# SouthPoleTelescope/CosmoMC

Hardware: AMD Instinct MI355X
Metric: fast-param likelihood evals/sec/node (plik_lite_TTTEEE ℓmax=2508); R-1 vs wall-clock (higher is better)
Workload: dtype f64; 1 GPU; plik_lite_TTTEEE + Planck2018 lensing fast-parameter Metropolis step (BASELINE configs[2] minus lowl): GetProposalFast + native plik_lite (613 bins, l<=2508, full binning + quadratic form) + CMBlikes lensing (9 bins, linear correction) + calPlanck prior + accept; walkers_per_gpu=1024, stream_groups=1, global_walkers=1024, nbins=613, lmax=2508, parallelism=walkers sharded over 1 rank(s), no per-step collective

## Files before the change

### cosmomc_amd/csrc/common.h

```cpp
#pragma once

#include <hip/hip_runtime.h>
#include <hip/hip_ext.h>

#include <algorithm>
#include <cstdarg>
#include <cstdint>
#include <cstdio>
#include <map>
#include <memory>
#include <mutex>
#include <stdexcept>
#include <string>
#include <vector>

#include "../../include/cosmomc_amd.h"

namespace cmamd {

struct Error : std::runtime_error {
    int code;
    Error(int c, const std::string &m) : std::runtime_error(m), code(c) {}
};

// ... 146 lines not shown
struct QFSource {
    const double *Ct = nullptr;
    int Np = 0, xcd_map = 0;
    const QFItem *items = nullptr;
    int n_items = 0;
    double *partial = nullptr;
    const double *X = nullptr;
    const double *delta = nullptr;
    unsigned int *counters = nullptr;
    int n_counters = 0;
};

struct SmallGaussDev {
    int nE, nX, has_corr, cal_index;
    double log_cal_prior;
    const int *e_to_x;
    const double *e_main_const, *e_corr_const;
    const double *fidcorr, *chat;
    int ntask;
    const int *trow;
    const int *e_main_t, *e_corr_t;
    const int *wcount;
};
struct SmallGaussLaunch {
    SmallGaussDev d;
    const double *partial;
    const double *nuis;
    long long ld_nuis;
    const double *M;
    double *out;
    int W;
    const unsigned char *row_cal;
    int stage_cal;
};

struct WinCol {
    int field, lo, hi;
    const double *w;
    int row;
    int cal;
};
struct WinStage {
    int kind = 0;
    int cal_index = -1;
    std::vector<WinCol> cols;
    const double *X = nullptr;
    int ld = 0;
};

struct Like {
    virtual ~Like() = default;
    std::string name, tag, nuisance_names;
    int n_nuis = 0;
    std::string derived_names;
    int n_derived = 0;
    virtual void derived_batch(int W, const double *nuis, long long ld_nuis, double *out, long long ld_out,
                               hipStream_t stream) {
        (void)nuis, (void)ld_nuis;
        if (W <= 0 || n_derived <= 0) return;
        if (!out || ld_out < n_derived) fail(CMBL_ERR_ARG, "derived output needs %d columns", n_derived);
        HIP_CHECK(hipMemset2DAsync(out, (size_t)ld_out * 8, 0, (size_t)n_derived * 8, W, stream));
    }
    const double *nuisance_rows(const double *nuis, const void *unread) const {
        if (n_nuis > 0 && !nuis) fail(CMBL_ERR_ARG, "%s needs its %d nuisance parameters", name.c_str(), n_nuis);
        return nuis ? nuis : static_cast<const double *>(unread);
    }
// ... 104 lines not shown
```

### cosmomc_amd/csrc/mhbody.h

```cpp
#pragma once

template <bool ACCEPT, bool PROPOSE>
__device__ __forceinline__ void mh_body(const DevCfg &c, int fast_only, double *hist_row, double *hist_terms, int blk0,
                                        double *lds, int bx, const TailWait *tw = nullptr)
{
    if (c.lean.on) {
        mh_lean<ACCEPT, PROPOSE>(c, hist_row, hist_terms, blk0, lds, bx, tw);
        return;
    }
    const Rows &R = c.rows;
    const int lane = threadIdx.x % MB, grp = threadIdx.x / MB;
    const int wl64 = threadIdx.x & 63, wave = threadIdx.x >> 6, nwave = MH_THREADS / 64;
    const int wb = (blk0 + bx) * MB;
    const int w = wb + lane;
    const bool act = w < c.W;
    const size_t W = c.ld;
    const int nlk = (c.n_like + 1) & ~1;
    const int nd_st = c.stage_R ? R.ND : R.ND - R.RR;
    const int ni_st = c.stage_cyc ? R.NI : R.CYC;
    const int ntd = c.stage_cov ? c.tl.n_dbl : c.tl.covinv;
    double *sd = lds;
    double *lk = sd + (size_t)nd_st * MB;
    double *vc = lk + (size_t)nlk * MB;
    double *tq = vc + (size_t)c.max_blk * MB;
    double *dq = tq + (size_t)c.tq_rows * MB;
    double *td = dq + (size_t)c.def_cap * (QF_GROUPS + 1) * MB;
    int *si = reinterpret_cast<int *>(td + ((ntd + 31) & ~31));
    int *it = si + (size_t)ni_st * MB;
    int *ti = it + (size_t)(c.stage_cyc ? c.all_n : 0) * MB;
    int *oobw = ti + ((c.tl.n_int + 63) & ~63);
    double *zz = reinterpret_cast<double *>(oobw + MB);
    int *ndw = reinterpret_cast<int *>(zz + (size_t)c.np * MB);
    int *i0w = ndw + MB;
    if (threadIdx.x < MB) oobw[threadIdx.x] = 0;
    if (PROPOSE && c.rot_defer && bx == 0 && threadIdx.x == 0)
        c.rot_cnt[2 * (blk0 * MB / 64) + (c.rot_par ^ 1)] = 0;
    const bool skipR = !c.stage_R;
#define SROW(r) ((skipR && (r) >= R.R) ? (r) - R.RR : (r))

    STAMP(0);
// ... 288 lines not shown
    }
    if (PROPOSE && c.pub_on && threadIdx.x < MB && act)
        for (int k = 0; k < 2; k++) {
            const int pc = c.pub_pcal[k];
            const bool rp = si[(size_t)R.PROT * MB + lane] != 0;
            const double v = rp ? __longlong_as_double((long long)TP_PIPE_ROT)
                                : pc >= 0 ? sd[(size_t)(SROW(R.T) + pc) * MB + lane] : 1.0;
            __hip_atomic_store(c.calbuf + (size_t)k * W + w, v, __ATOMIC_RELAXED, __HIP_MEMORY_SCOPE_AGENT);
            __hip_atomic_store(c.calbuf_next + (size_t)k * W + w, __longlong_as_double((long long)TP_PIPE_UNSET),
                               __ATOMIC_RELAXED, __HIP_MEMORY_SCOPE_AGENT);
        }
    if (act) {
        const int nd = ndw[lane], i0 = i0w[lane];
        for (int t = grp; t < nd; t += NV) {
            int p = i0 - 1 - t;
            if (p < 0) p += 97;
            c.sd[(size_t)(R.U + p) * W + w] = sd[(size_t)(R.U + p) * MB + lane];
        }
    }
    if (skipR) {
        stage_out(c.sd, sd, R.C, R.C, R.R, W, wb);
        stage_out(c.sd, sd, R.R, rEnd, R.ND, W, wb);
    } else {
        stage_out(c.sd, sd, R.C, R.C, R.ND, W, wb);
    }
    stage_out(c.si, si, 0, 0, ni_st, W, wb);
    STAMP(5);
#ifdef CMAMD_STAMPS
    asm volatile("s_waitcnt vmcnt(0)" ::: "memory");
    STAMP(6);
#endif
#undef SROW
}
```

### cosmomc_amd/csrc/mhlean.h

```cpp
#pragma once

template <bool ACCEPT, bool PROPOSE>
__device__ __forceinline__ void mh_lean(const DevCfg &c, double *hist_row, double *hist_terms, int blk0, double *lds,
                                        int bx, const TailWait *tw)
{
    const Rows &R = c.rows;
    const LeanCfg &L = c.lean;
    const int lane = threadIdx.x % MB, grp = threadIdx.x / MB;
    const int wl64 = threadIdx.x & 63, wave = threadIdx.x >> 6, nwave = MH_THREADS / 64;
    const int wb = (blk0 + bx) * MB;
    const int w = wb + lane;
    const bool act = w < c.W;
    const size_t W = c.ld;
    const int np = c.np;
    const int nd_lo = R.R, nd_hi = R.ND - R.P;
    double *sd = lds;
    double *sp = sd + (size_t)nd_lo * MB;
    double *dq = sp + (size_t)nd_hi * MB;
    double *zz = dq + (size_t)MAXDEF * (QF_GROUPS + 1) * MB;
    int *si = reinterpret_cast<int *>(zz + (size_t)np * MB);
    int *oobw = si + 8 * MB;
    int *ndw = oobw + MB;
    int *i0w = ndw + MB;
    if (threadIdx.x < MB) oobw[threadIdx.x] = 0;
    if (PROPOSE && c.rot_defer && bx == 0 && threadIdx.x == 0)
        c.rot_cnt[2 * (blk0 * MB / 64) + (c.rot_par ^ 1)] = 0;

    STAMP(0);
    dma_rows_f64(sd, 0, c.sd, 0, nd_lo, W, wb, wl64, wave, nwave);
    dma_rows_f64(sd, nd_lo, c.sd, R.P, nd_hi, W, wb, wl64, wave, nwave);
    dma_rows_i32(si, c.si, 8, W, wb, wl64, wave, nwave);
    constexpr int PG = MAXP / NV;
    double lo[PG], hi[PG], mu[PG], sg[PG];
    const double *td = c.tab_d;
#pragma unroll
    for (int u = 0; u < PG; u++) {
        const int i = grp + u * NV;
        if (ACCEPT && i < np) {
            lo[u] = td[c.tl.pmin + i];
            hi[u] = td[c.tl.pmax + i];
            mu[u] = td[c.tl.pmean + i];
            sg[u] = td[c.tl.pstd + i];
        }
    }
    int pu[PG];
    if (ACCEPT && hist_row) {
#pragma unroll
        for (int u = 0; u < PG; u++) {
            const int i = grp + u * NV;
            if (i < c.n_used) pu[u] = c.tab_i[c.tl.params_used + i];
        }
    }
    if (tw) tail_wait(*tw, wb / 64);
    if (ACCEPT && c.n_def) {
        const int tile = wb / QF_TILE, col = wb % QF_TILE + lane;
        for (int d = 0; d < MAXDEF; d++) {
            if (d >= c.n_def) break;
            const double *tp = c.def_part[d] + (size_t)tile * c.def_items[d] * QF_TILE;
            double *row = dq + (size_t)d * (QF_GROUPS + 1) * MB;
            if (grp < QF_GROUPS) row[(size_t)grp * MB + lane] = qf_group_sum(tp, c.def_items[d], grp, col);
            if (grp == NV - 1) row[(size_t)QF_GROUPS * MB + lane] = (c.def_add[d] && act) ? c.def_add[d][w] : 0.0;
        }
    }
    double lk[MAXLIKE], ct[MAXLIKE];
    if (ACCEPT && grp == 0 && act) {
#pragma unroll
        for (int l = 0; l < MAXLIKE; l++)
            if (l < c.n_like) {
                lk[l] = c.like_terms[(size_t)l * W + w];
                if (hist_terms) ct[l] = c.cur_terms[(size_t)l * W + w];
            }
    }
    STAMP(1);
    asm volatile("s_waitcnt vmcnt(0)" ::: "memory");
    __syncthreads();
    const double *trial_l = sp + (size_t)np * MB + lane;
    if (ACCEPT && act) {
        int oob = 0;
#pragma unroll
        for (int u = 0; u < PG; u++) {
            const int i = grp + u * NV;
            if (i < np) {
                const double qv = trial_l[(size_t)i * MB];
                if (qv > hi[u] || qv < lo[u]) oob = 1;
                double z2 = 0.0;
// ... 142 lines not shown
        c.si[(size_t)R.J97 * W + w] = r.j97;
        c.si[(size_t)R.ISET * W + w] = r.iset;
        ndw[lane] = r.nd < 97 ? r.nd : 97;
        i0w[lane] = i97_0;
    }
    __syncthreads();
    STAMP(12);
    if (!act) return;
    {
        const int nd = ndw[lane], i0 = i0w[lane];
        for (int t = grp; t < nd; t += NV) {
            int p = i0 - 1 - t;
            if (p < 0) p += 97;
            c.sd[(size_t)(R.U + p) * W + w] = sd[(size_t)(R.U + p) * MB + lane];
        }
    }
    for (int i = grp; i < np; i += NV) {
        if (ACCEPT) c.sd[(size_t)(R.P + i) * W + w] = sp[(size_t)i * MB + lane];
        if (PROPOSE) c.sd[(size_t)(R.T + i) * W + w] = sp[(size_t)(np + i) * MB + lane];
    }
    if (ACCEPT && hist_row) {
#pragma unroll
        for (int u = 0; u < PG; u++) {
            const int i = grp + u * NV;
            if (i < c.n_used) hist_row[(size_t)i * c.W + w] = sp[(size_t)pu[u] * MB + lane];
        }
    }
    STAMP(5);
#ifdef CMAMD_STAMPS
    asm volatile("s_waitcnt vmcnt(0)" ::: "memory");
    STAMP(6);
#endif
}
```

### cosmomc_amd/csrc/mhstep.h

```cpp
#pragma once


static constexpr int UNI_WT = 4;

template <bool ACCEPT, bool PROPOSE>
__device__ __forceinline__ void mh_step_body(DevCfg &c, int fast_only, double *hist_row, double *hist_terms,
                                             StepTail &t, const int2 *__restrict__ rows, TailWait &tw, int nmh)
{
    extern __shared__ __attribute__((aligned(16))) double lds[];
    const int2 rr = rows[blockIdx.x >> 3];
    const int lb = rr.y * 8 + (blockIdx.x & 7);
    if (!ACCEPT && blockIdx.x == 0)
        for (int i = threadIdx.x; i < tw.ntiles; i += MH_THREADS) tw.cnt[i] = 0u;
#ifdef CMAMD_STAMPS
    const bool stamp = ACCEPT && threadIdx.x == 0 && blockIdx.x < 2048;
    const int slot = PROPOSE ? 0 : 1;
    if (stamp) {
        unsigned xcc;
        asm volatile("s_getreg_b32 %0, hwreg(HW_REG_XCC_ID)" : "=s"(xcc));
        g_uni_stamps[slot][blockIdx.x][0] = __builtin_amdgcn_s_memrealtime();
        g_uni_stamps[slot][blockIdx.x][2] = xcc & 15;
        g_uni_stamps[slot][blockIdx.x][4] = 0;
        g_uni_stamps[slot][blockIdx.x][5] = 0;
    }
    struct End {
        bool on;
        int role, slot;
        __device__ ~End() {
            if (on) {
                g_uni_stamps[slot][blockIdx.x][3] = __builtin_amdgcn_s_memrealtime();
                g_uni_stamps[slot][blockIdx.x][4] = role + 1;
            }
        }
    } end_{stamp, rr.x, slot};
#endif
    if (rr.x == TAIL_QF) {
        if (lb >= t.nq) return;
        int item_ix, tile;
        qf_place(lb, t.q.src.n_items, t.q.src.xcd_map, item_ix, tile);
        __builtin_amdgcn_s_setprio(2);
        qfs_body(lds, item_ix, tile, t.q);
        tail_arrive(tw, tile);
    } else if (rr.x == TAIL_GAUSS) {
        const int grows = (t.ng + 7) >> 3, q = (lb & 7) * grows + (lb >> 3);
        if (q >= t.ng) return;
        small_gauss_body<UNI_WT, true, true>(t.g, lds, q);
        tail_arrive(tw, q * UNI_WT / 64);
    } else if (rr.x == TAIL_PASS) {
        if (lb >= t.np) return;
        tp_vec_body<2, true, false>(t.tp, t.dl, t.ld_field, t.ld_walker, t.W, reinterpret_cast<char *>(lds), lb);
    } else if (lb < nmh) {
        __builtin_amdgcn_s_setprio(3);
        if (ACCEPT && t.fold_g) {
            small_gauss_body<MB, true, false>(t.g, lds, lb);
            asm volatile("s_waitcnt vmcnt(0)" ::: "memory");
            __syncthreads();
#ifdef CMAMD_STAMPS
            if (threadIdx.x == 0 && blockIdx.x < 2048)
                g_uni_stamps[PROPOSE ? 0 : 1][blockIdx.x][5] = __builtin_amdgcn_s_memrealtime();
#endif
        }
        mh_body<ACCEPT, PROPOSE>(c, fast_only, hist_row, hist_terms, 0, lds, lb, ACCEPT ? &tw : nullptr);
    }
}
```

### cosmomc_amd/csrc/sampler.h

```cpp
#pragma once

#include "common.h"
#include "steptail.h"
#include "theorypass.h"

namespace cmamd {

static constexpr int MAXLIKE = 8;
static constexpr int MAXGROUPS = 8;
static constexpr int MAXDEF = 2;

struct Rows {
    int U = 0;
    int C = 97;
    int G = 98;
    int R = 100;
    int RR;
    int P, T, L, M;
    int ND;
    int I97 = 0, J97 = 1, ISET = 2, FASTIX = 3, NACC = 4;
    int CYCLP = 5;
    int BLKLP = 8;
    int ACCF;
    int PROT;
// ... 87 lines not shown
};

struct LikeSlot {
    cmbl_t *like;
    std::vector<int> nidx;
    TheoryView th;
};

struct PendingDeferred {
    int n = 0;
    int like[MAXDEF], items[MAXDEF];
    const double *part[MAXDEF], *add[MAXDEF];
};

struct PipeStatus {
    int *host = nullptr;
    int *dev = nullptr;
    hipEvent_t ev = nullptr;
    bool pending = false;
    void init();
    void post(hipStream_t stream);
    void post_nothrow(hipStream_t stream);
    void check(bool wait);
    ~PipeStatus() {
        if (host) (void)hipHostFree(host);
        if (ev) (void)hipEventDestroy(ev);
    }
};

struct UnifiedSteps {
    int ready = 0;
    DevBuf S[2][2];
    DevBuf rowcal;
    int qf = -1, g = -1;
    DevBuf cnt;
    size_t cnt_bytes = 0;
    unsigned epoch = 0;
    unsigned epoch_g = 0;
    StepTailPlan plan[3];
    size_t lds = 0;
    bool binned_cache = false;
    void invalidate() { ready = 0; }
};

struct BinCorun {
    int ready = 0;
    DevBuf cal;
    unsigned epoch = 0;
    DevBuf S;
    size_t lds = 0;
    void invalidate() { ready = 0; }
};

}

struct cmbg;

struct cmbs {
    cmamd::DevCfg dc{};
    int W = 0, np = 0, n_used = 0;
    std::vector<int> params_used;
    std::string last_error;
    cmamd::DevBuf rot;
    std::vector<int> rot_par;
    std::vector<int> rot_lp;
    bool rot_fast_any = false;
// ... 88 lines not shown
```

### cosmomc_amd/csrc/sampler.hip

```cpp
#include <algorithm>
#include <cmath>
#include <cstring>

#include <cstdlib>

#include "plikbin.h"
#include "qfs_body.h"
#include "quadform.h"
#include "sampler.h"
#include "smallgauss.h"
#include "theorycalc.h"
#ifdef CMAMD_STAMPS
namespace cmamd {
__device__ unsigned long long g_uni_stamps[2][2048][6];
}
#endif
#include "theorypass_body.h"

namespace cmamd {

static constexpr double LOGZERO = CMBL_LOGZERO;
static constexpr int MAXP = 64;
static constexpr int MAXBLK = 32;
static constexpr int NB = 64;
// ... 86 lines not shown
            }
            __builtin_amdgcn_s_sleep(24);
        }
        cal_s = cl;
    }
    __syncthreads();
    const double cl = cal_s, c2 = cl * cl;
    const bool rot = (unsigned long long)__double_as_longlong(cl) == TP_PIPE_ROT;
    double *out = (rot ? const_cast<double *>(c.bin_S) : c.bin_delta) + (size_t)w * pb.Np;
#pragma unroll
    for (int f = 0; f < 3; f++)
#pragma unroll
        for (int k = 0; k < 2; k++) {
            const int i = pb.fr.b0[f] + (int)threadIdx.x + k * MH_THREADS;
            if (pb.fr.hi[f] >= pb.fr.lo[f] && i < pb.fr.b1[f]) out[i] = rot ? acc[f][k] : pb.X[i] - acc[f][k] / c2;
        }
}

#include "mhstep.h"

template <bool ACCEPT, bool PROPOSE>
__global__ __launch_bounds__(MH_THREADS, 3) void mh_step_kernel(DevCfg c, int fast_only, double *hist_row,
                                                                double *hist_terms, StepTail t,
                                                                const int2 *__restrict__ rows, TailWait tw, int nmh)
{
    mh_step_body<ACCEPT, PROPOSE>(c, fast_only, hist_row, hist_terms, t, rows, tw, nmh);
}

template <bool ACCEPT, bool PROPOSE>
__global__ __launch_bounds__(MH_THREADS, 3) void mh_tail_kernel(DevCfg c, int fast_only, double *hist_row,
                                                                double *hist_terms, StepTail t,
                                                                const int2 *__restrict__ rows, TailWait tw, int nmh)
{
    mh_step_body<ACCEPT, PROPOSE>(c, fast_only, hist_row, hist_terms, t, rows, tw, nmh);
}

#include "mhrot.h"
#include "mhdrag.h"

__global__ void start_kernel(DevCfg c)
{
    const int w = blockIdx.x * blockDim.x + threadIdx.x;
    if (w >= c.W) return;
    const size_t W = c.ld;
    const Tabs t = make_tabs(c, c.tab_i, c.tab_d);
    Col<double> q{c.sd + (size_t)c.rows.T * W + w, c.ld};
    Col<const double> lk{c.like_terms + w, c.ld};
    c.sd[(size_t)c.rows.L * W + w] = target_like(c, t, q, lk);
    for (int l = 0; l < c.n_like; l++) c.cur_terms[(size_t)l * W + w] = lk[l];
    for (int i = 0; i < c.np; i++) c.sd[(size_t)(c.rows.P + i) * W + w] = q[i];
    c.sd[(size_t)c.rows.M * W + w] = 0.0;
    c.si[(size_t)c.rows.NACC * W + w] = 0;
}

__global__ void gather_nuis(const double *trial, int W, int ld, const int *nidx, int n_nuis, double *out)
{
    const int w = blockIdx.x * blockDim.x + threadIdx.x;
    if (w >= W) return;
    for (int k = 0; k < n_nuis; k++) out[(size_t)w * n_nuis + k] = trial[(size_t)nidx[k] * ld + w];
}

struct SparseSet {
    int like[MAXLIKE], nn[MAXLIKE];
    double *nuisc[MAXLIKE];
    int *map[MAXLIKE];
};

// ... 878 lines not shown
    return 0;
}
extern "C" int cmamd_debug_lean(cmbs *s, int on) {
    if (!s) return CMBL_ERR_ARG;
    s->lean_off = !on;
    return 0;
}
extern "C" int cmamd_debug_corun(cmbs *s, int on) {
    if (!s) return -1;
    s->no_corun = !on;
    return 0;
}
extern "C" int cmamd_debug_tail_nosignal(cmbs *s, int on) {
    if (!s) return -1;
    s->handoff_nosignal = on;
    return 0;
}
extern "C" int cmamd_debug_drag_pair(cmbs *s, int on) {
    if (!s) return -1;
    s->no_drag_pair = on == 0;
    return 0;
}
extern "C" int cmamd_debug_drag_hbm(cmbs *s, int on) {
    if (!s) return -1;
    s->drag_hbm = on != 0;
    return 0;
}
extern "C" int cmamd_debug_pipe_status(cmbs *s) {
    if (!s || !s->pipe_status.host) return -1;
    if (hipDeviceSynchronize() != hipSuccess) return -1;
    return *reinterpret_cast<volatile int *>(s->pipe_status.host);
}
extern "C" int cmamd_debug_tail(const cmbs *s) { return s ? s->unified.ready : 0; }
extern "C" int cmamd_debug_fused(const cmbs *s) { return !s ? 0 : s->tpass ? s->tpass->n_items() : -s->tp_why; }
```

### cosmomc_amd/csrc/schedunified.h

```cpp

using StepKernel = void (*)(DevCfg, int, double *, double *, StepTail, const int2 *, TailWait, int);
static const StepKernel step_kernels[2][3] = {
    {mh_step_kernel<false, true>, mh_step_kernel<true, true>, mh_step_kernel<true, false>},
    {mh_step_kernel<false, true>, mh_tail_kernel<true, true>, mh_tail_kernel<true, false>}};
static const char *const step_names[2][3] = {{"mh_step_first", "mh_step_kernel", "mh_step_last"},
                                             {"mh_step_first", "mh_tail_kernel", "mh_tail_last"}};

static bool unified_setup(cmbs *s, int fast_only) {
    if (s->sched_mode == 0 || !fast_only || !s->tpass || s->n_groups != 1 || s->mask_on ||
        (s->dc.rot_defer && s->rot_fast_any) || s->likes.size() != 2 || !s->dlikes.empty())
        return false;
    const TheoryView &P = s->likes[s->tp_like[0]].th;
    if (!s->tpass->vec_ok(P.dl, P.ld_field, P.ld_walker)) return false;
    UnifiedSteps &u = s->unified;
    if (u.ready == s->W) return true;
    if (u.ready == -s->W) return false;
    u.qf = u.g = -1;
    SmallGaussLaunch g{};
    for (int k = 0; k < 2; k++) {
        const int i = s->tp_like[k];
        const WinStage &st = s->tp_stage[k];
        QFSource src;
        if (st.kind == 1 && is_deferred(s, (size_t)i) && s->likes[i].like->like->qf_source(src, s->W, s->like_ws[i].p)) {
            bool all_cal = st.cal_index >= 0;
            for (const WinCol &c : st.cols) all_cal = all_cal && c.cal;
            if (all_cal && st.ld == src.Np) u.qf = k;
        }
        if (st.kind == 0 && small_gauss_on(s, trial_set(s), i, g)) u.g = k;
    }
    if (u.qf < 0 || u.g < 0 || u.qf == u.g) {
        u.ready = -s->W;
        return false;
    }
    const size_t Wp = (size_t)QuadForm::wpad(s->W);
    int rows = 0;
    for (const WinCol &c : s->tp_stage[u.g].cols) rows = std::max(rows, c.row + 1);
    const size_t bytes[2] = {Wp * (size_t)s->tp_stage[u.qf].ld * 8, (size_t)rows * s->W * 8};
    for (int p = 0; p < 2; p++)
        for (int k = 0; k < 2; k++) u.S[p][k].alloc(bytes[k == u.qf ? 0 : 1]);
    std::vector<unsigned char> rc((size_t)rows + 16, 0);
    for (const WinCol &c : s->tp_stage[u.g].cols) rc[c.row] = c.cal ? 1 : 0;
    u.rowcal.alloc(rc.size());
    u.rowcal.upload(rc.data(), rc.size());
    u.cnt_bytes = (Wp / QF_TILE * TW_PAD * 4 + 15) & ~(size_t)15;
    u.cnt.alloc(u.cnt_bytes);
    s->pipe_status.init();
    u.lds = std::max({s->mh_lds, (size_t)QFS_LDS_DOUBLES * 8, (size_t)tp_vec_lds_bytes<2>(),
                      (size_t)small_gauss_lds_doubles<UNI_WT>(g.d.nX) * 8,
                      (size_t)small_gauss_lds_doubles<MB>(g.d.nX) * 8});
    for (auto &ks : step_kernels)
        for (StepKernel k : ks)
            HIP_CHECK(hipFuncSetAttribute((const void *)k, hipFuncAttributeMaxDynamicSharedMemorySize, (int)u.lds));
    for (auto &pl : u.plan) pl.key[0] = -1;
    u.ready = s->W;
    return true;
}

static bool fold_chi2(bool has_pass, int nX) { return has_pass && nX <= MH_THREADS / MB; }

static StepTail make_tail(cmbs *s, int rd, int wr) {
    const UnifiedSteps &u = s->unified;
    StepTail t;
    const int W = s->W;
    t.W = W;
    if (rd >= 0) {
        const int qi = s->tp_like[u.qf];
        Like &Q = *s->likes[qi].like->like;
        if (!Q.qf_source(t.q.src, W, s->like_ws[qi].p)) fail(CMBL_ERR_ARG, "internal: step tail quadratic form");
        t.q.S = u.S[rd][u.qf].as<double>();
        t.q.nuis = s->dc.like_nuis[qi];
        t.q.ld_nuis = std::max(1, Q.n_nuis);
        t.q.cal_index = s->tp_stage[u.qf].cal_index;
        t.q.W = W;
        t.q.Wp = QuadForm::wpad(W);
        t.nq = t.q.src.n_items * (QuadForm::wpad(W) / QF_TILE);
        if (!small_gauss_on(s, trial_set(s), s->tp_like[u.g], t.g)) fail(CMBL_ERR_ARG, "internal: step tail chi^2");
        t.g.partial = u.S[rd][u.g].as<double>();
        t.g.row_cal = u.rowcal.as<unsigned char>();
        t.g.stage_cal = s->tp_stage[u.g].cal_index;
        t.fold_g = fold_chi2(wr >= 0, t.g.d.nX) ? 1 : 0;
        t.ng = t.fold_g ? 0 : (W + UNI_WT - 1) / UNI_WT;
    }
    if (wr >= 0) {
        TPOut o[2];
        fused_outs(s, trial_set(s), o, u.S[wr]);
        t.tp = s->tpass->dev_args(o, W);
        const TheoryView &P = s->likes[s->tp_like[0]].th;
        t.dl = P.dl;
        t.ld_field = P.ld_field;
        t.ld_walker = P.ld_walker;
        t.np = s->tpass->n_blocks();
    }
    return t;
}

static void launch_unified(cmbs *s, hipStream_t stream, bool propose, int rd, int wr, const HistRow &row,
                           int fast_only) {
    UnifiedSteps &u = s->unified;
    const bool accept = rd >= 0;
    StepTail t = make_tail(s, rd, wr);
    DevCfg dc = launch_cfg(s, fast_only, false);
    dc.n_def = accept ? 1 : 0;
    if (accept) {
        dc.def_like[0] = s->tp_like[u.qf];
        dc.def_items[0] = t.q.src.n_items;
        dc.def_part[0] = t.q.src.partial;
        dc.def_add[0] = nullptr;
    }
    TailWait tw{};
    tw.cnt = u.cnt.as<unsigned int>();
    tw.epoch = u.epoch + (accept ? 1u : 0u);
    tw.epoch_g = u.epoch_g + ((accept && !t.fold_g) ? 1u : 0u);
    tw.nq_items = t.q.src.n_items;
    tw.ng = accept ? (s->W + UNI_WT - 1) / UNI_WT : 0;
    tw.gwt = UNI_WT;
    tw.status = s->pipe_status.dev;
    tw.nosignal = s->handoff_nosignal;
    tw.stamp_slot = propose ? 0 : 1;
    tw.ntiles = (int)(u.cnt_bytes / 4);
    const int nmh = (s->W + MB - 1) / MB;
    const int v = accept ? (propose ? 1 : 2) : 0;
    StepTailPlan &pl = u.plan[v];
    if (pl.key[0] != t.nq || pl.key[1] != t.ng || pl.key[2] != t.np) {
        const std::vector<int2> rows = tail_rows(t.nq, t.ng, t.np, nmh);
        pl.d_rows.alloc(rows.size() * sizeof(int2));
        pl.d_rows.upload(rows.data(), rows.size() * sizeof(int2));
        pl.nrows = (int)rows.size();
        pl.key[0] = t.nq;
        pl.key[1] = t.ng;
        pl.key[2] = t.np;
    }
    const dim3 grid((unsigned)pl.nrows * 8), b(MH_THREADS);
    const int2 *rows = pl.d_rows.as<int2>();
    const bool cached = u.binned_cache && accept && wr < 0 && rd == 0;
    try {
        timed_launch(step_names[cached][v], stream, [&](hipEvent_t e0, hipEvent_t e1) {
            hipExtLaunchKernelGGL(step_kernels[cached][v], grid, b, u.lds, stream, e0, e1, 0, dc, fast_only, row.p,
                                  row.t, t, rows, tw, nmh);
        });
        HIP_CHECK(hipGetLastError());
    } catch (...) {
        u.invalidate();
        s->pipe_status.post_nothrow(stream);
        throw;
    }
    if (accept) u.epoch++;
    if (accept && !t.fold_g) u.epoch_g++;
}

static void run_unified(cmbs *s, int n_steps, int fast_only, hipStream_t stream) {
    s->unified.epoch = 0;
    s->unified.epoch_g = 0;
    launch_unified(s, stream, true, -1, 0, HistRow{}, fast_only);
    for (int k = 0; k < n_steps; k++) {
        const bool more = k + 1 < n_steps;
        if (s->unified.binned_cache) launch_unified(s, stream, more, 0, -1, next_hist(s), fast_only);
        else launch_unified(s, stream, more, k % 2, more ? (k + 1) % 2 : -1, next_hist(s), fast_only);
    }
    s->pipe_status.post(stream);
}
```

### cosmomc_amd/csrc/smallgauss.h

```cpp
#pragma once

#include "common.h"
#include "divrn.h"

namespace cmamd {

static constexpr int SMALL_NX = 64;
static constexpr int SMALL_WT = 4;
static constexpr int SMALL_MAXTASK = 256;

template <int WT> constexpr int small_gauss_lds_doubles() {
    return SMALL_MAXTASK * WT + SMALL_NX * WT + 256 + SMALL_NX * SMALL_NX;
}
template <int WT> constexpr int small_gauss_lds_doubles(int nX) {
    return SMALL_MAXTASK * WT + SMALL_NX * WT + 256 + nX * nX;
}

__device__ __forceinline__ int small_gauss_group(int lb, int ng)
{
    return (lb & 7) * ((ng + 7) >> 3) + (lb >> 3);
}
__host__ __device__ inline int small_gauss_blocks(int ng) { return (ng + 7) & ~7; }

template <int WT, bool RAWCAL = false, bool SIGNAL = false>
__device__ __forceinline__ void small_gauss_body(const SmallGaussLaunch &a, double *lds, int blk)
{
    constexpr int NG = 256 / WT;
    double *tp = lds;
    double *xs = tp + SMALL_MAXTASK * WT;
    double *red = xs + SMALL_NX * WT;
    double *Msh = red + NG * WT;
    const SmallGaussDev &c = a.d;
    const int W = a.W;
    const int wl = threadIdx.x % WT, g = threadIdx.x / WT;
    const int w = blk * WT + wl;
    const int Wc = c.wcount ? min(W, *c.wcount) : W;
    if (blk * WT >= Wc) return;
    for (int i = threadIdx.x; i < c.nX * c.nX; i += 256) Msh[i] = a.M[i];
    const bool act = w < Wc;
    const bool calp = c.log_cal_prior > 0 && c.cal_index >= 0;
    const double cal = (g == 0 && act && calp) ? a.nuis[(long long)w * a.ld_nuis + c.cal_index] : 1.0;
    double c2 = 1.0, rc2 = 1.0;
    if (RAWCAL && act && a.stage_cal >= 0) {
        const double cl = a.nuis[(long long)w * a.ld_nuis + a.stage_cal];
        c2 = cl * cl;
        rc2 = 1.0 / c2;
    }
    struct Elem { int ix, m0, m1, c0, c1; double mc, cc, fc, ch; };
    auto elem = [&](int e) {
        Elem q{c.e_to_x[e], c.e_main_t[e], c.e_main_t[e + 1], 0, 0, c.e_main_const[e], 0.0, 0.0, c.chat[e]};
        if (c.has_corr) {
            q.c0 = c.e_corr_t[e];
            q.c1 = c.e_corr_t[e + 1];
            q.cc = c.e_corr_const[e];
            q.fc = c.fidcorr[e];
        }
        return q;
    };
    Elem e0{-1, 0, 0, 0, 0, 0.0, 0.0, 0.0, 0.0};
    if (g < c.nE) e0 = elem(g);
    for (int t = g; t < c.ntask; t += NG) {
        const int4 ra = *reinterpret_cast<const int4 *>(c.trow + 8 * t);
        const int4 rb = *reinterpret_cast<const int4 *>(c.trow + 8 * t + 4);
        const int r[8] = {ra.x, ra.y, ra.z, ra.w, rb.x, rb.y, rb.z, rb.w};
        double v[8];
#pragma unroll
        for (int u = 0; u < 8; u++) v[u] = (act && r[u] >= 0) ? a.partial[(long long)r[u] * W + w] : 0.0;
        if (RAWCAL)
#pragma unroll
            for (int u = 0; u < 8; u++)
                if (r[u] >= 0 && a.row_cal[r[u]]) v[u] = div_rn(v[u], c2, rc2);
        double s = 0.0;
#pragma unroll
        for (int u = 0; u < 8; u++) s += v[u];
        tp[t * WT + wl] = s;
    }
    __syncthreads();
    for (int e = g; e < c.nE; e += NG) {
        const Elem q = e == g ? e0 : elem(e);
        if (q.ix < 0) continue;
        double s = q.mc;
        for (int t = q.m0; t < q.m1; t++) s += tp[t * WT + wl];
        if (c.has_corr) {
            double cs = q.cc;
            for (int t = q.c0; t < q.c1; t++) cs += tp[t * WT + wl];
            s = s + (cs - q.fc);
        }
        xs[q.ix * WT + wl] = s - q.ch;
    }
    __syncthreads();
    double part = 0.0;
    for (int i = g; i < c.nX; i += NG) {
        double y = 0.0;
        for (int j = 0; j < c.nX; j++) y += Msh[i * c.nX + j] * xs[j * WT + wl];
        part += xs[i * WT + wl] * y;
    }
    red[g * WT + wl] = part;
    __syncthreads();
    if (g == 0 && act) {
        double chisq = 0.0;
        for (int k = 0; k < NG; k++) chisq += red[k * WT + wl];
        if (calp) {
            const double t = log(cal) / c.log_cal_prior;
            chisq = chisq + t * t;
        }
        if (SIGNAL)
            __hip_atomic_store(a.out + w, chisq / 2, __ATOMIC_RELAXED, __HIP_MEMORY_SCOPE_AGENT);
        else
// ... 6 lines not shown
```

### cosmomc_amd/csrc/steptail.h

```cpp
#pragma once

#include <vector>

#include "common.h"
#include "theorypass.h"

namespace cmamd {

struct QFSArgs {
    QFSource src;
    const double *S;
    const double *nuis;
    long long ld_nuis;
    int cal_index;
    int W;
    int Wp;
};

struct StepTail {
    QFSArgs q;
    int nq = 0;
    SmallGaussLaunch g{};
    int ng = 0;
    int fold_g = 0;
    TPDev tp{};
    const double *dl = nullptr;
    long long ld_field = 0, ld_walker = 0;
    int np = 0;
    int W = 0;
};

enum { TAIL_QF = 0, TAIL_GAUSS = 1, TAIL_PASS = 2, TAIL_MH = 3 };
std::vector<int2> tail_rows(int nq, int ng, int np, int nm);

struct StepTailPlan {
    DevBuf d_rows;
    int key[3] = {-1, -1, -1};
    int nrows = 0;
};

}
```

Measured before the change: 32.48 million evals/s.

## Overlap lean MH staging with folded chi² and batch its partial loads

In the middle (accept+propose) launch, the lean MH stage loads (state rows, prior tables) are now issued before the folded small-Gaussian chi² runs, which uses LDS at an offset so the two do not collide. The folded chi² gains a batched form: the task row map and calibration flags are staged in LDS, and global partial loads for several tasks are issued together to hide memory latency. The covariance matrix load is overlapped with those reads. The theory-pass body is also instantiated with the MID flag. This raises LDS use and register pressure, and adds a debug query entry point.

```diff
diff --git a/cosmomc_amd/csrc/common.h b/cosmomc_amd/csrc/common.h
--- a/cosmomc_amd/csrc/common.h
+++ b/cosmomc_amd/csrc/common.h
@@ -202,6 +202,7 @@
     int W;
     const unsigned char *row_cal;
     int stage_cal;
+    int n_rowcal;
 };
 
 struct WinCol {
diff --git a/cosmomc_amd/csrc/mhbody.h b/cosmomc_amd/csrc/mhbody.h
--- a/cosmomc_amd/csrc/mhbody.h
+++ b/cosmomc_amd/csrc/mhbody.h
@@ -2,10 +2,10 @@
 
 template <bool ACCEPT, bool PROPOSE>
 __device__ __forceinline__ void mh_body(const DevCfg &c, int fast_only, double *hist_row, double *hist_terms, int blk0,
-                                        double *lds, int bx, const TailWait *tw = nullptr)
+                                        double *lds, int bx, const TailWait *tw, LeanStage &S, bool staged)
 {
     if (c.lean.on) {
-        mh_lean<ACCEPT, PROPOSE>(c, hist_row, hist_terms, blk0, lds, bx, tw);
+        mh_lean<ACCEPT, PROPOSE>(c, hist_row, hist_terms, blk0, lds, bx, tw, S, staged);
         return;
     }
     const Rows &R = c.rows;
@@ -360,3 +360,11 @@
 #endif
 #undef SROW
 }
+
+template <bool ACCEPT, bool PROPOSE>
+__device__ __forceinline__ void mh_body(const DevCfg &c, int fast_only, double *hist_row, double *hist_terms, int blk0,
+                                        double *lds, int bx, const TailWait *tw = nullptr)
+{
+    LeanStage S;
+    mh_body<ACCEPT, PROPOSE>(c, fast_only, hist_row, hist_terms, blk0, lds, bx, tw, S, false);
+}
diff --git a/cosmomc_amd/csrc/mhlean.h b/cosmomc_amd/csrc/mhlean.h
--- a/cosmomc_amd/csrc/mhlean.h
+++ b/cosmomc_amd/csrc/mhlean.h
@@ -1,56 +1,95 @@
 #pragma once
 
+struct LeanStage {
+    static constexpr int PG = MAXP / NV;
+    double lo[PG], hi[PG], mu[PG], sg[PG];
+    int pu[PG];
+};
+
+struct LeanLds {
+    double *sd, *sp, *dq, *zz;
+    int *si, *oobw, *ndw, *i0w;
+    int nd_lo, nd_hi;
+    __device__ __forceinline__ LeanLds(const DevCfg &c, double *lds)
+    {
+        const Rows &R = c.rows;
+        nd_lo = R.R;
+        nd_hi = R.ND - R.P;
+        sd = lds;
+        sp = sd + (size_t)nd_lo * MB;
+        dq = sp + (size_t)nd_hi * MB;
+        zz = dq + (size_t)MAXDEF * (QF_GROUPS + 1) * MB;
+        si = reinterpret_cast<int *>(zz + (size_t)c.np * MB);
+        oobw = si + 8 * MB;
+        ndw = oobw + MB;
+        i0w = ndw + MB;
+    }
+};
+
 template <bool ACCEPT, bool PROPOSE>
-__device__ __forceinline__ void mh_lean(const DevCfg &c, double *hist_row, double *hist_terms, int blk0, double *lds,
-                                        int bx, const TailWait *tw)
+__device__ __forceinline__ void mh_lean_stage(const DevCfg &c, double *hist_row, int blk0, double *lds, int bx,
+                                              LeanStage &S)
+{
+    const Rows &R = c.rows;
+    const int grp = threadIdx.x / MB;
+    const int wl64 = threadIdx.x & 63, wave = threadIdx.x >> 6, nwave = MH_THREADS / 64;
+#ifdef CMAMD_STAMPS
+    const int lane = threadIdx.x % MB;
+#endif
+    const int wb = (blk0 + bx) * MB;
+    const size_t W = c.ld;
+    const int np = c.np;
+    const LeanLds I(c, lds);
+    if (threadIdx.x < MB) I.oobw[threadIdx.x] = 0;
+    if (PROPOSE && c.rot_defer && bx == 0 && threadIdx.x == 0)
+        c.rot_cnt[2 * (blk0 * MB / 64) + (c.rot_par ^ 1)] = 0;
+
+    STAMP(0);
+    dma_rows_f64(I.sd, 0, c.sd, 0, I.nd_lo, W, wb, wl64, wave, nwave);
+    dma_rows_f64(I.sd, I.nd_lo, c.sd, R.P, I.nd_hi, W, wb, wl64, wave, nwave);
+    dma_rows_i32(I.si, c.si, 8, W, wb, wl64, wave, nwave);
+    constexpr int PG = LeanStage::PG;
+    const double *td = c.tab_d;
+#pragma unroll
+    for (int u = 0; u < PG; u++) {
+        const int i = grp + u * NV;
+        if (ACCEPT && i < np) {
+            S.lo[u] = td[c.tl.pmin + i];
+            S.hi[u] = td[c.tl.pmax + i];
+            S.mu[u] = td[c.tl.pmean + i];
+            S.sg[u] = td[c.tl.pstd + i];
+        }
+    }
+    if (ACCEPT && hist_row) {
+#pragma unroll
+        for (int u = 0; u < PG; u++) {
+            const int i = grp + u * NV;
+            if (i < c.n_used) S.pu[u] = c.tab_i[c.tl.params_used + i];
+        }
+    }
+}
+
+template <bool ACCEPT, bool PROPOSE>
+__device__ __forceinline__ void mh_lean_chain(const DevCfg &c, double *hist_row, double *hist_terms, int blk0,
+                                              double *lds, int bx, const TailWait *tw, const LeanStage &S)
 {
     const Rows &R = c.rows;
     const LeanCfg &L = c.lean;
     const int lane = threadIdx.x % MB, grp = threadIdx.x / MB;
-    const int wl64 = threadIdx.x & 63, wave = threadIdx.x >> 6, nwave = MH_THREADS / 64;
+#ifdef CMAMD_STAMPS
+    const int wave = threadIdx.x >> 6;
+#endif
     const int wb = (blk0 + bx) * MB;
     const int w = wb + lane;
     const bool act = w < c.W;
     const size_t W = c.ld;
     const int np = c.np;
-    const int nd_lo = R.R, nd_hi = R.ND - R.P;
-    double *sd = lds;
-    double *sp = sd + (size_t)nd_lo * MB;
-    double *dq = sp + (size_t)nd_hi * MB;
-    double *zz = dq + (size_t)MAXDEF * (QF_GROUPS + 1) * MB;
-    int *si = reinterpret_cast<int *>(zz + (size_t)np * MB);
-    int *oobw = si + 8 * MB;
-    int *ndw = oobw + MB;
-    int *i0w = ndw + MB;
-    if (threadIdx.x < MB) oobw[threadIdx.x] = 0;
-    if (PROPOSE && c.rot_defer && bx == 0 && threadIdx.x == 0)
-        c.rot_cnt[2 * (blk0 * MB / 64) + (c.rot_par ^ 1)] = 0;
-
-    STAMP(0);
-    dma_rows_f64(sd, 0, c.sd, 0, nd_lo, W, wb, wl64, wave, nwave);
-    dma_rows_f64(sd, nd_lo, c.sd, R.P, nd_hi, W, wb, wl64, wave, nwave);
-    dma_rows_i32(si, c.si, 8, W, wb, wl64, wave, nwave);
-    constexpr int PG = MAXP / NV;
-    double lo[PG], hi[PG], mu[PG], sg[PG];
-    const double *td = c.tab_d;
-#pragma unroll
-    for (int u = 0; u < PG; u++) {
-        const int i = grp + u * NV;
-        if (ACCEPT && i < np) {
-            lo[u] = td[c.tl.pmin + i];
-            hi[u] = td[c.tl.pmax + i];
-            mu[u] = td[c.tl.pmean + i];
-            sg[u] = td[c.tl.pstd + i];
-        }
-    }
-    int pu[PG];
-    if (ACCEPT && hist_row) {
-#pragma unroll
-        for (int u = 0; u < PG; u++) {
-            const int i = grp + u * NV;
-            if (i < c.n_used) pu[u] = c.tab_i[c.tl.params_used + i];
-        }
-    }
+    const LeanLds I(c, lds);
+    double *const sd = I.sd, *const sp = I.sp, *const dq = I.dq, *const zz = I.zz;
+    int *const si = I.si, *const oobw = I.oobw, *const ndw = I.ndw, *const i0w = I.i0w;
+    constexpr int PG = LeanStage::PG;
+    const double *const lo = S.lo, *const hi = S.hi, *const mu = S.mu, *const sg = S.sg;
+    const int *const pu = S.pu;
     if (tw) tail_wait(*tw, wb / 64);
     if (ACCEPT && c.n_def) {
         const int tile = wb / QF_TILE, col = wb % QF_TILE + lane;
@@ -259,3 +298,11 @@
     STAMP(6);
 #endif
 }
+
+template <bool ACCEPT, bool PROPOSE>
+__device__ __forceinline__ void mh_lean(const DevCfg &c, double *hist_row, double *hist_terms, int blk0, double *lds,
+                                        int bx, const TailWait *tw, LeanStage &S, bool staged)
+{
+    if (!staged) mh_lean_stage<ACCEPT, PROPOSE>(c, hist_row, blk0, lds, bx, S);
+    mh_lean_chain<ACCEPT, PROPOSE>(c, hist_row, hist_terms, blk0, lds, bx, tw, S);
+}
diff --git a/cosmomc_amd/csrc/mhstep.h b/cosmomc_amd/csrc/mhstep.h
--- a/cosmomc_amd/csrc/mhstep.h
+++ b/cosmomc_amd/csrc/mhstep.h
@@ -3,7 +3,7 @@
 
 static constexpr int UNI_WT = 4;
 
-template <bool ACCEPT, bool PROPOSE>
+template <bool ACCEPT, bool PROPOSE, bool MID = ACCEPT && PROPOSE>
 __device__ __forceinline__ void mh_step_body(DevCfg &c, int fast_only, double *hist_row, double *hist_terms,
                                              StepTail &t, const int2 *__restrict__ rows, TailWait &tw, int nmh)
 {
@@ -38,6 +38,9 @@
         if (lb >= t.nq) return;
         int item_ix, tile;
         qf_place(lb, t.q.src.n_items, t.q.src.xcd_map, item_ix, tile);
+#ifdef CMAMD_STAMPS
+        if (stamp) g_uni_stamps[slot][blockIdx.x][2] |= (unsigned)(tile + 1) << 8;
+#endif
         __builtin_amdgcn_s_setprio(2);
         qfs_body(lds, item_ix, tile, t.q);
         tail_arrive(tw, tile);
@@ -48,18 +51,34 @@
         tail_arrive(tw, q * UNI_WT / 64);
     } else if (rr.x == TAIL_PASS) {
         if (lb >= t.np) return;
-        tp_vec_body<2, true, false>(t.tp, t.dl, t.ld_field, t.ld_walker, t.W, reinterpret_cast<char *>(lds), lb);
+        tp_vec_body<2, true, MID>(t.tp, t.dl, t.ld_field, t.ld_walker, t.W, reinterpret_cast<char *>(lds), lb);
     } else if (lb < nmh) {
         __builtin_amdgcn_s_setprio(3);
-        if (ACCEPT && t.fold_g) {
-            small_gauss_body<MB, true, false>(t.g, lds, lb);
-            asm volatile("s_waitcnt vmcnt(0)" ::: "memory");
-            __syncthreads();
 #ifdef CMAMD_STAMPS
-            if (threadIdx.x == 0 && blockIdx.x < 2048)
-                g_uni_stamps[PROPOSE ? 0 : 1][blockIdx.x][5] = __builtin_amdgcn_s_memrealtime();
+        if (stamp) g_uni_stamps[slot][blockIdx.x][2] |= (unsigned)(lb * MB / 64 + 1) << 8;
 #endif
+        if constexpr (MID) {
+            LeanStage ls;
+            bool staged = false;
+            if (t.fold_g) {
+                if (t.pre_off) mh_lean_stage<ACCEPT, PROPOSE>(c, hist_row, 0, lds, lb, ls);
+                small_gauss_body<MB, true, false, UNI_FOLD_B>(t.g, lds + t.pre_off, lb);
+                asm volatile("s_waitcnt vmcnt(0)" ::: "memory");
+                __syncthreads();
+#ifdef CMAMD_STAMPS
+                if (threadIdx.x == 0 && blockIdx.x < 2048)
+                    g_uni_stamps[PROPOSE ? 0 : 1][blockIdx.x][5] = __builtin_amdgcn_s_memrealtime();
+#endif
+                staged = t.pre_off != 0;
+            }
+            mh_body<ACCEPT, PROPOSE>(c, fast_only, hist_row, hist_terms, 0, lds, lb, ACCEPT ? &tw : nullptr, ls, staged);
+        } else {
+            if (ACCEPT && t.fold_g) {
+                small_gauss_body<MB, true, false>(t.g, lds, lb);
+                asm volatile("s_waitcnt vmcnt(0)" ::: "memory");
+                __syncthreads();
+            }
+            mh_body<ACCEPT, PROPOSE>(c, fast_only, hist_row, hist_terms, 0, lds, lb, ACCEPT ? &tw : nullptr);
         }
-        mh_body<ACCEPT, PROPOSE>(c, fast_only, hist_row, hist_terms, 0, lds, lb, ACCEPT ? &tw : nullptr);
     }
 }
diff --git a/cosmomc_amd/csrc/sampler.h b/cosmomc_amd/csrc/sampler.h
--- a/cosmomc_amd/csrc/sampler.h
+++ b/cosmomc_amd/csrc/sampler.h
@@ -143,6 +143,8 @@
     int ready = 0;
     DevBuf S[2][2];
     DevBuf rowcal;
+    int n_rowcal = 0;
+    int mid_fold_g = 0, mid_pre_off = 0;
     int qf = -1, g = -1;
     DevBuf cnt;
     size_t cnt_bytes = 0;
diff --git a/cosmomc_amd/csrc/sampler.hip b/cosmomc_amd/csrc/sampler.hip
--- a/cosmomc_amd/csrc/sampler.hip
+++ b/cosmomc_amd/csrc/sampler.hip
@@ -142,7 +142,7 @@
                                                                 double *hist_terms, StepTail t,
                                                                 const int2 *__restrict__ rows, TailWait tw, int nmh)
 {
-    mh_step_body<ACCEPT, PROPOSE>(c, fast_only, hist_row, hist_terms, t, rows, tw, nmh);
+    mh_step_body<ACCEPT, PROPOSE, false>(c, fast_only, hist_row, hist_terms, t, rows, tw, nmh);
 }
 
 #include "mhrot.h"
@@ -1087,4 +1087,11 @@
     return *reinterpret_cast<volatile int *>(s->pipe_status.host);
 }
 extern "C" int cmamd_debug_tail(const cmbs *s) { return s ? s->unified.ready : 0; }
+extern "C" int cmamd_debug_fold_chi2(cmbs *s, int *out) {
+    try {
+        return s && out && cmamd::fold_info(s, out) ? 0 : -1;
+    } catch (...) {
+        return -5;
+    }
+}
 extern "C" int cmamd_debug_fused(const cmbs *s) { return !s ? 0 : s->tpass ? s->tpass->n_items() : -s->tp_why; }
diff --git a/cosmomc_amd/csrc/schedunified.h b/cosmomc_amd/csrc/schedunified.h
--- a/cosmomc_amd/csrc/schedunified.h
+++ b/cosmomc_amd/csrc/schedunified.h
@@ -38,16 +38,17 @@
     const size_t bytes[2] = {Wp * (size_t)s->tp_stage[u.qf].ld * 8, (size_t)rows * s->W * 8};
     for (int p = 0; p < 2; p++)
         for (int k = 0; k < 2; k++) u.S[p][k].alloc(bytes[k == u.qf ? 0 : 1]);
-    std::vector<unsigned char> rc((size_t)rows + 16, 0);
+    std::vector<unsigned char> rc(((size_t)rows + 16 + 3) & ~(size_t)3, 0);
     for (const WinCol &c : s->tp_stage[u.g].cols) rc[c.row] = c.cal ? 1 : 0;
     u.rowcal.alloc(rc.size());
     u.rowcal.upload(rc.data(), rc.size());
+    u.n_rowcal = (int)rc.size();
     u.cnt_bytes = (Wp / QF_TILE * TW_PAD * 4 + 15) & ~(size_t)15;
     u.cnt.alloc(u.cnt_bytes);
     s->pipe_status.init();
     u.lds = std::max({s->mh_lds, (size_t)QFS_LDS_DOUBLES * 8, (size_t)tp_vec_lds_bytes<2>(),
                       (size_t)small_gauss_lds_doubles<UNI_WT>(g.d.nX) * 8,
-                      (size_t)small_gauss_lds_doubles<MB>(g.d.nX) * 8});
+                      (size_t)small_gauss_batched_lds_doubles(MB, g.d.ntask, g.d.nX, u.n_rowcal) * 8});
     for (auto &ks : step_kernels)
         for (StepKernel k : ks)
             HIP_CHECK(hipFuncSetAttribute((const void *)k, hipFuncAttributeMaxDynamicSharedMemorySize, (int)u.lds));
@@ -77,6 +78,7 @@
         if (!small_gauss_on(s, trial_set(s), s->tp_like[u.g], t.g)) fail(CMBL_ERR_ARG, "internal: step tail chi^2");
         t.g.partial = u.S[rd][u.g].as<double>();
         t.g.row_cal = u.rowcal.as<unsigned char>();
+        t.g.n_rowcal = u.n_rowcal;
         t.g.stage_cal = s->tp_stage[u.g].cal_index;
         t.fold_g = fold_chi2(wr >= 0, t.g.d.nX) ? 1 : 0;
         t.ng = t.fold_g ? 0 : (W + UNI_WT - 1) / UNI_WT;
@@ -94,6 +96,30 @@
     return t;
 }
 
+static int fold_pre_off(const cmbs *s, const StepTail &t, const DevCfg &dc) {
+    if (!t.fold_g || !dc.lean.on) return 0;
+    const size_t off = (lean_lds_bytes(s) + 15) & ~(size_t)15;
+    const size_t need = (size_t)small_gauss_batched_lds_doubles(MB, t.g.d.ntask, t.g.d.nX, t.g.n_rowcal) * 8;
+    return off + need <= s->unified.lds ? (int)(off / 8) : 0;
+}
+
+static bool fold_info(cmbs *s, int out[5]) {
+    const UnifiedSteps &u = s->unified;
+    if (u.ready != s->W || u.g < 0) return false;
+    StepTail t;
+    if (!small_gauss_on(s, trial_set(s), s->tp_like[u.g], t.g)) return false;
+    t.g.n_rowcal = u.n_rowcal;
+    out[0] = t.g.d.ntask;
+    out[1] = UNI_FOLD_B;
+    out[2] = MH_THREADS / MB;
+    out[3] = u.mid_fold_g ? (u.mid_pre_off > 0 ? 2 : 1) : 0;
+    int last[8] = {-1, -1, -1, -1, -1, -1, -1, -1};
+    if (t.g.d.ntask > 0) HIP_CHECK(hipMemcpy(last, t.g.d.trow + 8 * (t.g.d.ntask - 1), sizeof(last), hipMemcpyDeviceToHost));
+    out[4] = 0;
+    for (int r : last) out[4] += r >= 0;
+    return true;
+}
+
 static void launch_unified(cmbs *s, hipStream_t stream, bool propose, int rd, int wr, const HistRow &row,
                            int fast_only) {
     UnifiedSteps &u = s->unified;
@@ -101,6 +127,7 @@
     StepTail t = make_tail(s, rd, wr);
     DevCfg dc = launch_cfg(s, fast_only, false);
     dc.n_def = accept ? 1 : 0;
+    t.pre_off = fold_pre_off(s, t, dc);
     if (accept) {
         dc.def_like[0] = s->tp_like[u.qf];
         dc.def_items[0] = t.q.src.n_items;
@@ -133,6 +160,11 @@
     const dim3 grid((unsigned)pl.nrows * 8), b(MH_THREADS);
     const int2 *rows = pl.d_rows.as<int2>();
     const bool cached = u.binned_cache && accept && wr < 0 && rd == 0;
+    if (t.fold_g && !(accept && propose && !cached)) fail(CMBL_ERR_ARG, "internal: a folded chi^2 outside the middle launch");
+    if (accept && propose) {
+        u.mid_fold_g = t.fold_g;
+        u.mid_pre_off = t.pre_off;
+    }
     try {
         timed_launch(step_names[cached][v], stream, [&](hipEvent_t e0, hipEvent_t e1) {
             hipExtLaunchKernelGGL(step_kernels[cached][v], grid, b, u.lds, stream, e0, e1, 0, dc, fast_only, row.p,
diff --git a/cosmomc_amd/csrc/smallgauss.h b/cosmomc_amd/csrc/smallgauss.h
--- a/cosmomc_amd/csrc/smallgauss.h
+++ b/cosmomc_amd/csrc/smallgauss.h
@@ -22,21 +22,41 @@
 }
 __host__ __device__ inline int small_gauss_blocks(int ng) { return (ng + 7) & ~7; }
 
-template <int WT, bool RAWCAL = false, bool SIGNAL = false>
+__host__ __device__ inline int small_gauss_batched_lds_doubles(int WT, int ntask, int nX, int n_rowcal)
+{
+    return 4 * ntask + ntask * WT + nX * WT + 256 + nX * nX + (n_rowcal + 7) / 8 + 1;
+}
+
+template <int WT, bool RAWCAL = false, bool SIGNAL = false, int B = 0>
 __device__ __forceinline__ void small_gauss_body(const SmallGaussLaunch &a, double *lds, int blk)
 {
+    static_assert(B == 0 || RAWCAL, "the batched form reads raw sums");
     constexpr int NG = 256 / WT;
-    double *tp = lds;
-    double *xs = tp + SMALL_MAXTASK * WT;
-    double *red = xs + SMALL_NX * WT;
+    const SmallGaussDev &c = a.d;
+    int *trs = reinterpret_cast<int *>(lds);
+    double *tp = B > 0 ? lds + 4 * c.ntask : lds;
+    double *xs = tp + (B > 0 ? c.ntask : SMALL_MAXTASK) * WT;
+    double *red = xs + (B > 0 ? c.nX : SMALL_NX) * WT;
     double *Msh = red + NG * WT;
-    const SmallGaussDev &c = a.d;
+    unsigned *rcs = reinterpret_cast<unsigned *>(Msh + c.nX * c.nX);
     const int W = a.W;
     const int wl = threadIdx.x % WT, g = threadIdx.x / WT;
     const int w = blk * WT + wl;
     const int Wc = c.wcount ? min(W, *c.wcount) : W;
     if (blk * WT >= Wc) return;
-    for (int i = threadIdx.x; i < c.nX * c.nX; i += 256) Msh[i] = a.M[i];
+    static_assert(SMALL_MAXTASK * 2 <= 512, "two int4 a thread stage trow");
+    int4 tra = make_int4(-1, -1, -1, -1), trb = tra;
+    unsigned rc4 = 0;
+    double m0 = 0.0;
+    if (B > 0) {
+        if ((int)threadIdx.x < 2 * c.ntask) tra = reinterpret_cast<const int4 *>(c.trow)[threadIdx.x];
+        if ((int)threadIdx.x + 256 < 2 * c.ntask) trb = reinterpret_cast<const int4 *>(c.trow)[threadIdx.x + 256];
+        if ((int)threadIdx.x < (a.n_rowcal + 3) / 4) rc4 = reinterpret_cast<const unsigned *>(a.row_cal)[threadIdx.x];
+        if ((int)threadIdx.x < c.nX * c.nX) m0 = a.M[threadIdx.x];
+        for (int i = threadIdx.x + 256; i < c.nX * c.nX; i += 256) Msh[i] = a.M[i];
+    } else {
+        for (int i = threadIdx.x; i < c.nX * c.nX; i += 256) Msh[i] = a.M[i];
+    }
     const bool act = w < Wc;
     const bool calp = c.log_cal_prior > 0 && c.cal_index >= 0;
     const double cal = (g == 0 && act && calp) ? a.nuis[(long long)w * a.ld_nuis + c.cal_index] : 1.0;
@@ -59,21 +79,66 @@
     };
     Elem e0{-1, 0, 0, 0, 0, 0.0, 0.0, 0.0, 0.0};
     if (g < c.nE) e0 = elem(g);
-    for (int t = g; t < c.ntask; t += NG) {
-        const int4 ra = *reinterpret_cast<const int4 *>(c.trow + 8 * t);
-        const int4 rb = *reinterpret_cast<const int4 *>(c.trow + 8 * t + 4);
-        const int r[8] = {ra.x, ra.y, ra.z, ra.w, rb.x, rb.y, rb.z, rb.w};
-        double v[8];
+    if (B > 0) {
+        if ((int)threadIdx.x < 2 * c.ntask) reinterpret_cast<int4 *>(trs)[threadIdx.x] = tra;
+        if ((int)threadIdx.x + 256 < 2 * c.ntask) reinterpret_cast<int4 *>(trs)[threadIdx.x + 256] = trb;
+        if ((int)threadIdx.x < (a.n_rowcal + 3) / 4) rcs[threadIdx.x] = rc4;
+        for (int i = threadIdx.x + 256; i < (a.n_rowcal + 3) / 4; i += 256)
+            rcs[i] = reinterpret_cast<const unsigned *>(a.row_cal)[i];
+        __syncthreads();
+        const unsigned char *rcb = reinterpret_cast<const unsigned char *>(rcs);
+        constexpr int NB = B > 0 ? B : 1;
+        for (int t0 = g; t0 < c.ntask; t0 += NG * NB) {
+            int r[NB][8];
+            double v[NB][8];
 #pragma unroll
-        for (int u = 0; u < 8; u++) v[u] = (act && r[u] >= 0) ? a.partial[(long long)r[u] * W + w] : 0.0;
-        if (RAWCAL)
+            for (int k = 0; k < NB; k++) {
+                const int t = t0 + k * NG;
+                int4 ra = make_int4(-1, -1, -1, -1), rb = ra;
+                if (t < c.ntask) {
+                    ra = *reinterpret_cast<const int4 *>(trs + 8 * t);
+                    rb = *reinterpret_cast<const int4 *>(trs + 8 * t + 4);
+                }
+                const int q[8] = {ra.x, ra.y, ra.z, ra.w, rb.x, rb.y, rb.z, rb.w};
 #pragma unroll
-            for (int u = 0; u < 8; u++)
-                if (r[u] >= 0 && a.row_cal[r[u]]) v[u] = div_rn(v[u], c2, rc2);
-        double s = 0.0;
+                for (int u = 0; u < 8; u++) r[k][u] = q[u];
+            }
 #pragma unroll
-        for (int u = 0; u < 8; u++) s += v[u];
-        tp[t * WT + wl] = s;
+            for (int k = 0; k < NB; k++)
+#pragma unroll
+                for (int u = 0; u < 8; u++)
+                    v[k][u] = (act && r[k][u] >= 0) ? a.partial[(long long)r[k][u] * W + w] : 0.0;
+            if (t0 == g && (int)threadIdx.x < c.nX * c.nX) Msh[threadIdx.x] = m0;
+#pragma unroll
+            for (int k = 0; k < NB; k++) {
+                const int t = t0 + k * NG;
+#pragma unroll
+                for (int u = 0; u < 8; u++)
+                    if (r[k][u] >= 0 && rcb[r[k][u]]) v[k][u] = div_rn(v[k][u], c2, rc2);
+                double s = 0.0;
+#pragma unroll
+                for (int u = 0; u < 8; u++) s += v[k][u];
+                if (t < c.ntask) tp[t * WT + wl] = s;
+            }
+        }
+        if (g >= c.ntask && (int)threadIdx.x < c.nX * c.nX) Msh[threadIdx.x] = m0;
+    } else {
+        for (int t = g; t < c.ntask; t += NG) {
+            const int4 ra = *reinterpret_cast<const int4 *>(c.trow + 8 * t);
+            const int4 rb = *reinterpret_cast<const int4 *>(c.trow + 8 * t + 4);
+            const int r[8] = {ra.x, ra.y, ra.z, ra.w, rb.x, rb.y, rb.z, rb.w};
+            double v[8];
+#pragma unroll
+            for (int u = 0; u < 8; u++) v[u] = (act && r[u] >= 0) ? a.partial[(long long)r[u] * W + w] : 0.0;
+            if (RAWCAL)
+#pragma unroll
+                for (int u = 0; u < 8; u++)
+                    if (r[u] >= 0 && a.row_cal[r[u]]) v[u] = div_rn(v[u], c2, rc2);
+            double s = 0.0;
+#pragma unroll
+            for (int u = 0; u < 8; u++) s += v[u];
+            tp[t * WT + wl] = s;
+        }
     }
     __syncthreads();
     for (int e = g; e < c.nE; e += NG) {
diff --git a/cosmomc_amd/csrc/steptail.h b/cosmomc_amd/csrc/steptail.h
--- a/cosmomc_amd/csrc/steptail.h
+++ b/cosmomc_amd/csrc/steptail.h
@@ -17,12 +17,15 @@
     int Wp;
 };
 
+static constexpr int UNI_FOLD_B = 4;
+
 struct StepTail {
     QFSArgs q;
     int nq = 0;
     SmallGaussLaunch g{};
     int ng = 0;
     int fold_g = 0;
+    int pre_off = 0;
     TPDev tp{};
     const double *dl = nullptr;
     long long ld_field = 0, ld_walker = 0;
```

After: 32.91 million evals/s, median of 6. 1.01x the previous value.
